# RL-VIG/LibContinual

Hardware: AMD Instinct MI355X
Metric: images/sec/node (task-0 epoch), CIFAR-100 B50-5x10 (higher is better)
Workload: dtype bf16; 1 GPU; lwf_resnet18_b50_task0; method=LWF, backbone=resnet18, per_gpu_batch=256, global_batch=256, image=3x32x32, parallelism=dp1, optimizer=fused SGD

## Files before the change

### libcontinual_amd/csrc/api.hip

```cpp
#include <map>
#include <utility>
#include <vector>
#include <mutex>
#include <string>
#include <string.h>
#include <stdio.h>
#include <stdlib.h>

#include "kernels.h"

static thread_local char g_err[512] = "";

void clhip_set_error(const char* fmt, ...) {
    va_list ap;
    va_start(ap, fmt);
    vsnprintf(g_err, sizeof(g_err), fmt, ap);
    va_end(ap);
}

extern "C" const char* clhip_last_error(void) { return g_err; }
extern "C" int clhip_version(void) { return 103; }

namespace {
const char* const kKeys[] = {
    "ATTN_GENERIC", "ATTN_BWD", "BN_FUSE", "BN_FUSE_MAX_M", "BN_MASK_BITS", "BN_MASK_FROM_Y", "BN_PARTIALS", "CE_ROWS", "CE_ONE_WG", "LINEAR_BWD_SPLIT", "CONV3G", "CONV4", "CONV_V1",
    "GEMM_NO_SPLIT", "GEMM_TAIL", "NO_CONV16", "NO_CONV3", "NO_PARITY_DGRAD", "NO_SHORTCUT", "NO_STEM", "PREP_NARROW", "WGRAD4",
    "WGRAD_NO_TR", "WGRAD2_ATOMIC", "WGRAD_DEFER", "WGRAD_DEFER_SIDE", "BWD_FUSED", "WGRAD_STREAM", "BRANCH_STREAM", "WGRAD_ALWAYS_QUEUE", "SIDE_PRIO", "EVENT_FLAGS", "EVENT_RECORD", "CONV5", "CONV6", "WGRAD16_PARTS", "WGRAD32_IPG", "WGRAD64_IPG", "WGRAD64_IPI2", "CONV64", "CONV64_BM", "CONV64_FWD", "CONV6_PAIR", "CONV7", "CONV7_TPW", "WGRAD7", "FWD7", "PAIR_BN_FUSE", "POOL_BN_FUSE", "BN_INPUT", "BN_INPUT_WT", "BN_RES_INPUT", "BN_GRAD", "BN_GRAD_MINC", "BN_GRAD_RES", "CONV6_DEBUG", "BN_ONEPASS", "WGRAD5", "WGRAD32",
    "BN_ACC_CPT", "BN_BWD_ITERS", "CONV3_CFG", "CONV4_CFG", "CONV4_GRID", "GEMM_GROUP_M", "GEMM_MT", "IGEMM_TILE",
    "SHORTCUT_MIN_PIXELS", "STEM_GRID", "STEM_WGRAD_GRID", "WGRAD4_MIN_STEPS", "WGRAD4_MIN_TOTAL", "WGRAD_NET_GFLOP", "WGRAD_TARGET",
    "CONV5_MIN_TILES", "CONV5_GRID", "CONV64_MAX_W", "CONV64_MAX_M", "CONV8", "CONV8_MIN_TILES", "DZ_BUFFERS", "CONV8_GRID", "CONV8_OPT", "CONV8_BNR", "CONV9", "PLAN_SKIP", "WT_DEBUG", "EVAL_LAZY", "GEMM_SPLITK", "STREAM_PROBE", "STAGE_EVAL", "STAGE_TRAIN", "STAGE_TRAIN_BWD", "STAGE_TRACE", "STAGE_ENTRY", "STAGE_ENTRY_BWD", "STAGE_POOL", "STAGE_XCH3", "ADAPTER_TM",
    "CONV3_DEBUG", "WGRAD_DEBUG", "CONV4_FORCE_CFG", "CONV4_ENABLE", "CONV4_DEBUG", "CONV4_TRACE", "WGRAD4_TRACE", "CONV6_TRACE", "CONV8_TRACE", "CONV9_TRACE",
};
std::mutex g_stream_mu;
std::mutex g_cfg_mu;
std::map<std::string, const char*>& cfg_map() { static std::map<std::string, const char*> m; return m; }
bool known_key(const char* k) {
    for (const char* q : kKeys) if (strcmp(q, k) == 0) return true;
    return false;
}
}

namespace {
__global__ void stream_probe_spin_kernel(unsigned long long* out, long long ticks) {
    const unsigned long long t0 = wall_clock64();
    while ((long long)(wall_clock64() - t0) < ticks) __builtin_amdgcn_s_sleep(64);
    out[0] = wall_clock64();
}
__global__ void stream_probe_stamp_kernel(unsigned long long* out) { out[1] = wall_clock64(); }

struct SharedStreams {
    std::vector<hipStream_t> pool;
    std::map<std::pair<hipStream_t, int>, hipStream_t> chosen;
    hipStream_t low_prio = nullptr;
    unsigned long long* probe_buf = nullptr;
};
SharedStreams g_shared[16];

bool runs_beside(SharedStreams& S, hipStream_t a, hipStream_t b) {
    if (S.probe_buf == nullptr && hipMalloc(reinterpret_cast<void**>(&S.probe_buf), 2 * sizeof(unsigned long long)) != hipSuccess) return false;
    hipLaunchKernelGGL(stream_probe_spin_kernel, dim3(1), dim3(1), 0, a, S.probe_buf, 30000ll);
    hipLaunchKernelGGL(stream_probe_stamp_kernel, dim3(1), dim3(1), 0, b, S.probe_buf);
    if (hipStreamSynchronize(b) != hipSuccess || hipStreamSynchronize(a) != hipSuccess) return false;
    unsigned long long h[2] = {0, 0};
// ... 106 lines not shown
```

### libcontinual_amd/csrc/conv.hip

```cpp
#include <stdlib.h>

#include <algorithm>

#include "kernels.h"

namespace {

constexpr int BK = 32;

struct ConvParams {
    const void* src;
    const void* wt;
    void* dst;
    float* stats;
    int N, Hs, Ws, Cs, log2Cs, Hd, Wd, Cd, ksize, stride, pad, accumulate;
    int M;
    int K;
};

template <typename T> struct Chunk;
template <> struct Chunk<bf16_t> { uint4 a; };
template <> struct Chunk<float> { uint4 a, b; };

template <typename T> __device__ __forceinline__ Chunk<T> zero_chunk() {
// ... 361 lines not shown
    int BN = Cd >= 128 ? 128 : (Cd >= 64 ? 64 : (Cd >= 32 ? 32 : 16));
    int gy = (Cd + BN - 1) / BN;
    bool small = ((int64_t)((M + 127) / 128) * gy) < 512;
    return small ? 64 : 128;
}

int check_conv(int N, int H, int W, int C, int K, int ksize, int stride, int pad) {
    CLHIP_CHECK_ARG(N > 0 && H > 0 && W > 0);
    CLHIP_CHECK_ARG(ksize == 1 || ksize == 3);
    CLHIP_CHECK_ARG(stride >= 1 && pad >= 0);
    CLHIP_CHECK_ARG(C >= 8 && ilog2_exact(C) >= 0);
    CLHIP_CHECK_ARG(K >= 16 && K % 16 == 0);
    CLHIP_CHECK_ARG((int64_t)N * H * W * (C > K ? C : K) < (int64_t)1 << 31);
    return CLHIP_OK;
}

}

static bool use_v3() {
    static const bool v = clhip_cfg("NO_CONV3") == nullptr;
    return v;
}
static bool use_v1() {
    static const bool v = clhip_cfg("CONV_V1") != nullptr;
    return v;
}

extern "C" int clhip_conv_fwd_tiles(int N, int H, int W, int C, int K, int ksize, int stride, int pad) {
    int Ho = (H + 2 * pad - ksize) / stride + 1, Wo = (W + 2 * pad - ksize) / stride + 1;
    int M = N * Ho * Wo;
    if (ksize == 7) return clhip_stem7_supported(N, H, W, C, K, stride, pad) ? clhip_stem7_fwd_tiles(N, H, W) : 0;
    if (!use_v1()) {
        int t2 = clhip_conv2_tiles_m(M, K);
        if (use_v3() && clhip_conv16_supported(H, W, C, K, ksize, stride, pad, CLHIP_BF16)) {
            int t16 = clhip_conv16_tiles_m(M);
            return t16 > t2 ? t16 : t2;
        }
        if (use_v3() && clhip_conv3_supported(H, W, C, K, ksize, stride, pad, CLHIP_BF16)) {
            int t3 = clhip_conv3_tiles_m(M, K);
            if (clhip_conv4_supported(N, H, W, C, K, ksize, stride, pad, CLHIP_BF16)) { int t4 = clhip_conv4_tiles_m(M, C, K, W); if (t4 > t3) t3 = t4; }
            return t3 > t2 ? t3 : t2;
        }
        return t2;
    }
    int bm = fwd_tile_m(M, K);
    return (M + bm - 1) / bm;
}

static bool conv64_fwd_on() { const char* c = clhip_cfg("CONV64_FWD"); return !(c != nullptr && atoi(c) == 0); }

static bool wgrad_v1_no_tr() { static const bool v = clhip_cfg("WGRAD_NO_TR") != nullptr; return v; }

enum { OP_FWD = 0, OP_DGRAD = 1, OP_WGRAD = 2, OP_DGRAD_BNR = 3, OP_FWD_WT = 4 };
static int route_conv(int op, int form, int N, int H, int W, int C, int Creal, int K, int ksize, int stride, int pad, int dtype) {
    CLHIP_CHECK_ARG(op >= OP_FWD && op <= OP_FWD_WT);
    CLHIP_CHECK_ARG(form >= 0 && form <= (op == OP_FWD ? 2 : (op == OP_WGRAD ? 1 : 0)));
    if (ksize == 7 && (op == OP_FWD || op == OP_WGRAD)) {
        CLHIP_CHECK_ARG(clhip_stem7_supported(N, H, W, C, K, stride, pad));
        if (op == OP_FWD) CLHIP_CHECK_ARG(form != 1);
        else CLHIP_CHECK_ARG(form == 1 && Creal >= 1 && Creal <= C && (K * 49 * Creal) % 4 == 0);
        CLHIP_CHECK_ARG(dtype == CLHIP_BF16 || dtype == CLHIP_F32);
        return op == OP_FWD ? CLHIP_CONV_STEM7 : CLHIP_CONV_WGRAD_STEM7;
    }
    if (int e = check_conv(N, H, W, C, K, ksize, stride, pad)) return e;
    const bool v2 = !use_v1();
    const bool v3 = v2 && use_v3();
    if (op == OP_FWD) {
        CLHIP_CHECK_ARG(!(form == 2 && !v2));
        CLHIP_CHECK_ARG(dtype == CLHIP_BF16 || dtype == CLHIP_F32);
        const bool rows = form == 1;
        if (v3 && !rows && clhip_stem_supported(N, H, W, C, K, ksize, stride, pad, dtype)) return CLHIP_CONV_STEM;
        if (v3 && !rows && conv64_fwd_on() && clhip_conv64_supported(N, H, W, C, K, ksize, stride, pad, dtype)) return CLHIP_CONV_CONV64;
        if (v3 && clhip_conv16_supported(H, W, C, K, ksize, stride, pad, dtype)) return CLHIP_CONV_CONV16;
        if (v3 && !rows && clhip_conv8_supported(N, H, W, C, K, ksize, stride, pad, dtype)) return CLHIP_CONV_CONV8;
        if (v3 && !rows && clhip_conv5_supported(N, H, W, C, K, ksize, stride, pad, dtype)) return CLHIP_CONV_CONV5;
        if (v3 && !rows && clhip_conv9_supported(N, H, W, C, K, ksize, stride, pad, dtype)) return CLHIP_CONV_CONV9;
        if (v3 && clhip_conv4_supported(N, H, W, C, K, ksize, stride, pad, dtype)) return CLHIP_CONV_CONV4;
        if (v3 && clhip_conv3_supported(H, W, C, K, ksize, stride, pad, dtype)) return CLHIP_CONV_CONV3;
        return v2 ? CLHIP_CONV_CONV2 : CLHIP_CONV_V1;
    }
    if (op == OP_DGRAD) {
        CLHIP_CHECK_ARG(C % 16 == 0);
        CLHIP_CHECK_ARG(ilog2_exact(K) >= 0);
        CLHIP_CHECK_ARG(dtype == CLHIP_BF16 || dtype == CLHIP_F32);
        if (v3 && clhip_shortcut_supported(N, H, W, C, K, ksize, stride, pad, dtype)) return CLHIP_CONV_SHORTCUT;
        if (v3 && clhip_conv16_supported(H, W, K, C, ksize, stride, pad, dtype)) return CLHIP_CONV_CONV16;
        if (v3 && clhip_conv64_supported(N, H, W, K, C, ksize, stride, pad, dtype)) return CLHIP_CONV_CONV64;
        if (v3 && clhip_conv8_supported(N, H, W, K, C, ksize, stride, pad, dtype)) return CLHIP_CONV_CONV8;
        if (v3 && clhip_conv5_supported(N, H, W, K, C, ksize, stride, pad, dtype)) return CLHIP_CONV_CONV5;
        if (v3 && clhip_conv9_supported(N, H, W, K, C, ksize, stride, pad, dtype)) return CLHIP_CONV_CONV9;
        if (v3 && clhip_conv4_supported(N, H, W, K, C, ksize, stride, pad, dtype)) return CLHIP_CONV_CONV4;
        if (v3 && clhip_conv3_supported(H, W, K, C, ksize, stride, pad, dtype)) return CLHIP_CONV_CONV3;
        return v2 ? CLHIP_CONV_CONV2 : CLHIP_CONV_V1;
    }
    if (op == OP_WGRAD) {
        CLHIP_CHECK_ARG(Creal >= 1 && Creal <= C);
        CLHIP_CHECK_ARG(dtype == CLHIP_BF16 || dtype == CLHIP_F32);
        const bool ws = form == 1;
        if (v3 && ws && clhip_stem_wgrad_supported(N, H, W, C, Creal, K, ksize, stride, pad, dtype)) return CLHIP_CONV_WGRAD_STEM;
        if (v3 && ws && clhip_wgrad64_supported(N, H, W, C, Creal, K, ksize, stride, pad, dtype)) return CLHIP_CONV_WGRAD64;
        if (v3 && ws && clhip_wgrad4_supported(N, H, W, C, Creal, K, ksize, stride, pad, dtype)) return CLHIP_CONV_WGRAD4;
        if (v3 && clhip_wgrad3_supported(N, H, W, C, Creal, K, ksize, stride, pad, dtype)) return CLHIP_CONV_WGRAD3;
        if (v3 && ws && clhip_wgrad16_supported(N, H, W, C, Creal, K, ksize, stride, pad, dtype)) return CLHIP_CONV_WGRAD16;
        if (v3 && ws && clhip_wgrad32_supported(N, H, W, C, Creal, K, ksize, stride, pad, dtype)) return CLHIP_CONV_WGRAD32;
        if (v2) return (ws && clhip_wgrad2_ws_bytes(N, H, W, C, Creal, K, ksize, stride, pad) > 0) ? CLHIP_CONV_WGRAD2_DET : CLHIP_CONV_WGRAD2_ATOMIC;
        return (dtype == CLHIP_BF16 && !wgrad_v1_no_tr()) ? CLHIP_CONV_WGRAD_V1 : CLHIP_CONV_WGRAD_V1_NO_TR;
    }
    if (op == OP_DGRAD_BNR) {
        CLHIP_CHECK_ARG(v3 && (clhip_conv16_supported(H, W, K, C, ksize, stride, pad, dtype) || clhip_conv64_supported(N, H, W, K, C, ksize, stride, pad, dtype) ||
                               clhip_conv8_supported(N, H, W, K, C, ksize, stride, pad, dtype) || clhip_conv4_supported(N, H, W, K, C, ksize, stride, pad, dtype)));
// ... 33 lines not shown
}

static int conv_fwd_impl(const void* x, const void* w_fwd, void* z, float* stat_partials, double* stat_acc, int stat_rep, int N, int H, int W, int C,
                         int K, int ksize, int stride, int pad, int dtype, void* stream) {
    const int family = route_conv(OP_FWD, stat_partials ? 1 : (stat_acc ? 2 : 0), N, H, W, C, C, K, ksize, stride, pad, dtype);
    if (family < 0) return family;
    CLHIP_CHECK_ARG(x && w_fwd && z);
    hipStream_t st = static_cast<hipStream_t>(stream);
    if (family == CLHIP_CONV_STEM7) return clhip_stem7_fwd_launch(x, w_fwd, z, stat_acc, stat_rep, N, H, W, K, dtype, st);
    ConvParams p;
    p.src = x; p.wt = w_fwd; p.dst = z; p.stats = stat_partials;
    p.N = N; p.Hs = H; p.Ws = W; p.Cs = C; p.log2Cs = ilog2_exact(C);
    p.Hd = (H + 2 * pad - ksize) / stride + 1; p.Wd = (W + 2 * pad - ksize) / stride + 1; p.Cd = K;
    p.ksize = ksize; p.stride = stride; p.pad = pad; p.accumulate = 0;
    p.M = N * p.Hd * p.Wd; p.K = ksize * ksize * C;
    ConvCall c;
    c.src = x; c.wt = w_fwd; c.dst = z; c.stats = stat_partials; c.stat_acc = stat_acc; c.stat_rep = stat_rep;
    c.N = N; c.H = H; c.W = W; c.Cs = C; c.Cd = K;
    auto zero_tail = [&](int tiles_used) {
        const int tiles_alloc = clhip_conv_fwd_tiles(N, H, W, C, K, ksize, stride, pad);
        if (stat_partials && tiles_alloc > tiles_used)
            hipMemsetAsync(stat_partials + (size_t)tiles_used * 2 * K, 0, (size_t)(tiles_alloc - tiles_used) * 2 * K * sizeof(float), st);
    };
    switch (family) {
        case CLHIP_CONV_STEM: return clhip_stem_launch(x, w_fwd, z, stat_acc, stat_rep, N, H, W, K, st);
        case CLHIP_CONV_CONV64: return clhip_conv64_launch(c, st);
        case CLHIP_CONV_CONV16:
            zero_tail(clhip_conv16_tiles_m(p.M));
            return clhip_conv16_launch(c, st);
        case CLHIP_CONV_CONV8: return clhip_conv8_launch(c, st);
        case CLHIP_CONV_CONV5: return clhip_conv5_launch(c, st);
        case CLHIP_CONV_CONV9: return clhip_conv9_launch(c, st);
        case CLHIP_CONV_CONV4:
            zero_tail(clhip_conv4_tiles_m(p.M, C, K, W));
            return clhip_conv4_launch(c, st);
        case CLHIP_CONV_CONV3:
            zero_tail(clhip_conv3_tiles_m(p.M, K));
            return clhip_conv3_launch(c, st);
        case CLHIP_CONV_CONV2:
            zero_tail(clhip_conv2_tiles_m(p.M, K));
            return clhip_conv2_launch(x, w_fwd, z, stat_partials, stat_acc, stat_rep, N, H, W, C, p.Hd, p.Wd, K, ksize, stride, pad, 0, 0, dtype, st);
        case CLHIP_CONV_V1: return dtype == CLHIP_BF16 ? launch_igemm<bf16_t, 0>(p, st) : launch_igemm<float, 0>(p, st);
        default: break;
    }
    clhip_set_error("clhip_conv_fwd: no launch for kernel family %d", family);
    return CLHIP_EINVAL;
}

extern "C" int clhip_conv_dgrad(const void* dz, const void* w_dg, void* dx, int accumulate, int N, int H, int W, int C,
                                int K, int ksize, int stride, int pad, int dtype, void* stream) {
    const int family = route_conv(OP_DGRAD, 0, N, H, W, C, C, K, ksize, stride, pad, dtype);
    if (family < 0) return family;
    CLHIP_CHECK_ARG(dz && w_dg && dx);
    ConvParams p;
    p.src = dz; p.wt = w_dg; p.dst = dx; p.stats = nullptr;
    p.N = N; p.Hs = (H + 2 * pad - ksize) / stride + 1; p.Ws = (W + 2 * pad - ksize) / stride + 1; p.Cs = K;
    p.log2Cs = ilog2_exact(K);
    p.Hd = H; p.Wd = W; p.Cd = C;
    p.ksize = ksize; p.stride = stride; p.pad = pad; p.accumulate = accumulate;
    p.M = N * H * W; p.K = ksize * ksize * K;
    ConvCall c;
    c.src = dz; c.wt = w_dg; c.dst = dx; c.N = N; c.H = H; c.W = W; c.Cs = K; c.Cd = C; c.accumulate = accumulate; c.mode = 1;
    hipStream_t st = static_cast<hipStream_t>(stream);
    switch (family) {
        case CLHIP_CONV_SHORTCUT: return clhip_shortcut_dgrad(dz, w_dg, dx, accumulate, N, H, W, C, K, st);
        case CLHIP_CONV_CONV16: return clhip_conv16_launch(c, st);
        case CLHIP_CONV_CONV64: return clhip_conv64_launch(c, st);
// ... 310 lines not shown
```

### libcontinual_amd/csrc/conv4.hip

```cpp
#include <stdlib.h>

#include "kernels.h"

namespace {

int g_force4[4] = {0, 0, 0, 0};
int g_enable4 = -1, g_debug4 = 0;
unsigned long long* g_trace4 = nullptr;

typedef __attribute__((ext_vector_type(16))) float f32x16;
typedef __attribute__((ext_vector_type(4))) unsigned u32x4;
typedef __attribute__((address_space(1))) const void gvoid_t;
typedef __attribute__((address_space(3))) void lvoid_t;

struct Conv4Params {
    const bf16_t* src;
    const bf16_t* wt;
    bf16_t* dst;
    float* stats;
    double* stat_acc;
    int stat_rep;
    const bf16_t* bn_z;
    const bf16_t* bn_y;
    const float* bn_mean;
    const float* bn_invstd;
    double* bn_acc;
    int bn_rep;
    int H, W, Cs, Cd, M, accumulate;
    int wshift, hshift;
    int np;
    int patch_bytes;
    int n_ntiles, nt_shift, n_items;
    int cpg;
    unsigned long long* trace;
    int debug;
};

template <int MODE>
__device__ __forceinline__ unsigned tap_mask4(int g, const Conv4Params& p) {
    int w, h;
    if (p.wshift >= 0 && p.hshift >= 0) { w = g & (p.W - 1); h = (g >> p.wshift) & (p.H - 1); }
    else { w = g % p.W; h = (g / p.W) % p.H; }
    constexpr unsigned UP = MODE == 0 ? 0x007u : 0x1c0u, DOWN = MODE == 0 ? 0x1c0u : 0x007u;
    constexpr unsigned LEFT = MODE == 0 ? 0x049u : 0x124u, RIGHT = MODE == 0 ? 0x124u : 0x049u;
    unsigned m = 0x1ffu;
    if (h == 0) m &= ~UP;
    if (h == p.H - 1) m &= ~DOWN;
    if (w == 0) m &= ~LEFT;
    if (w == p.W - 1) m &= ~RIGHT;
    return m;
}

#ifdef CLHIP_ABLATION
#define DBG(p) ((p).debug)
#define STAMP() do { if (p.trace && blockIdx.x == 0 && lane == 0 && (wave & 3) == 0 && nstamp < 256) p.trace[(wave >> 2) * 256 + nstamp++] = __builtin_amdgcn_s_memtime(); } while (0)
#else
#define STAMP() do { } while (0)
#define DBG(p) 0
#endif

template <int N> __device__ __forceinline__ void wait_vm() { __builtin_amdgcn_s_waitcnt((N & 15) | 0x70 | 0xF00 | ((N >> 4) << 14)); }
__device__ __forceinline__ void wait_lds() { __builtin_amdgcn_s_waitcnt(0xC07F); }
__device__ __forceinline__ void wg_barrier(bool skip = false) {
    wait_lds();
    if (!skip) __builtin_amdgcn_s_barrier();
    asm volatile("" ::: "memory");
}

template <int WM, int WN, int KG, int CK, int WMAX, int MODE>
__global__ __launch_bounds__(WM * WN * KG * 64, 2) void conv4_kernel(const Conv4Params p) {
    constexpr int BM = WM * 64, BN = WN * 64, NWG = WM * WN, NTG = NWG * 64;
    constexpr int NST = 3;
    constexpr int PP = CK * 2 + 16;
    constexpr int KS = CK / 16;
    constexpr int WROW = CK * 2;
    constexpr int SPR = WROW / 16;
    constexpr int RPI = 64 / SPR;
    constexpr int SLAB = BN * WROW;
    constexpr int WINST = (BN / RPI) / NWG;
    static_assert((BN / RPI) % NWG == 0 && WINST >= 1, "ring rows must divide among the waves of a group");
    constexpr int SPP = PP / 16;
    constexpr int ZBYTES = 512;
    constexpr int PINST = ((((BM + 2 * WMAX + 2) * PP + 255) / 256 * 256 + ZBYTES) / 1024 + 1 + NWG - 1) / NWG;
    constexpr int PL_TAP = 2;
    constexpr bool SETPRIO = false;
    constexpr bool STAG = NWG * KG == 8;

    extern __shared__ __attribute__((aligned(16))) char smem[];
    const int tid = threadIdx.x, lane = tid & 63;
    const int wave = __builtin_amdgcn_readfirstlane(tid >> 6);
    const int grp = wave / NWG, wv = wave % NWG;
    int nstamp = 0; (void)nstamp;
    const int wm = wv / WN, wn = wv % WN;
    const int l31 = lane & 31, kh = lane >> 5;
    const int W = p.W, Cs = p.Cs, halo = W + 1;
    const int K9 = 9 * Cs;

    char* patch_g = smem + grp * 2 * p.patch_bytes;
    char* ring0 = smem + KG * 2 * p.patch_bytes;
    char* ring_g = ring0 + grp * SLAB;
    constexpr int XR_BYTES = KG > 1 ? (KG - 1) * NWG * 64 * 64 * 4 : 0;
    const int ring_end = KG * 2 * p.patch_bytes + NST * KG * SLAB;
    float* red = reinterpret_cast<float*>(smem + (ring_end > XR_BYTES ? ring_end : XR_BYTES));

    int xaddr[2];
#pragma unroll
    for (int i = 0; i < 2; ++i) xaddr[i] = (wm * 64 + i * 32 + l31 + halo) * PP + kh * 16;
    const int zoff = (p.np * PP + 255) / 256 * 256;
    int waddr[2][KS];
#pragma unroll
    for (int j = 0; j < 2; ++j) {
        const int o = wn * 64 + j * 32 + l31;
        const int swz = CK == 64 ? ((o >> 1) & 7) : ((o >> 2) & 3);
#pragma unroll
        for (int ks = 0; ks < KS; ++ks) waddr[j][ks] = o * WROW + (((2 * ks + kh) ^ swz) << 4);
    }
    unsigned dma_lane[WINST];
#pragma unroll
    for (int i = 0; i < WINST; ++i) {
        const int row = (wv * WINST + i) * RPI + lane / SPR;
        const int slot = lane % SPR;
        const int swz = CK == 64 ? ((row >> 1) & 7) : ((row >> 2) & 3);
        dma_lane[i] = (unsigned)((row * K9 + (slot ^ swz) * 8) * 2);
    }
    const char* wbase = reinterpret_cast<const char*>(p.wt);
    auto dma = [&](int item, int cc, int tap, int stage) {
        const int n0 = (item & (p.n_ntiles - 1)) * BN;
        const size_t uni = ((size_t)n0 * K9 + (size_t)tap * Cs + (size_t)(grp * p.cpg + cc) * CK) * 2;
        const char* g = wbase + uni;
        char* l = ring_g + stage * (KG * SLAB) + wv * (WINST * 1024);
        if (DBG(p) & 2) return;
#if defined(__HIP_DEVICE_COMPILE__)
#pragma unroll
        for (int i = 0; i < WINST; ++i)
            __builtin_amdgcn_global_load_lds((gvoid_t*)(g + dma_lane[i]), (lvoid_t*)(l + i * 1024), 16, 0, 0);
#else
        (void)g; (void)l;
#endif
    };

    const __amdgpu_buffer_rsrc_t srs = __builtin_amdgcn_make_buffer_rsrc(const_cast<bf16_t*>(p.src), 0, p.M * Cs * 2, 0x00020000);
    constexpr int OOB = 0x40000000;
    int prel[PINST];
#pragma unroll
    for (int i = 0; i < PINST; ++i) {
        const int slot = (wv * PINST + i) * 64 + lane;
        const int q = slot / SPP, sub = slot - q * SPP;
        prel[i] = (q < p.np && sub < SPP - 1) ? q * (Cs * 2) + sub * 16 : OOB;
    }
    auto pdma = [&](int item, int cc, int buf) {
        const int m0 = (item >> p.nt_shift) * BM;
        const int base = (m0 - halo) * (Cs * 2) + (grp * p.cpg + cc) * CK * 2;
        char* l = patch_g + buf * p.patch_bytes + wv * (PINST * 1024);
#if defined(__HIP_DEVICE_COMPILE__)
#pragma unroll
        for (int i = 0; i < PINST; ++i)
            __builtin_amdgcn_raw_ptr_buffer_load_lds(srs, (lvoid_t*)(l + i * 1024), 16, prel[i] + base, 0, 0, 0);
#else
        (void)base; (void)l;
#endif
    };

    const int G = gridDim.x;
    const int nmy = (p.n_items - (int)blockIdx.x + G - 1) / G;
    const int cpg = p.cpg;

    const bool pl_on = !(DBG(p) & 4);
    if (pl_on) pdma(blockIdx.x, 0, 0);
    dma(blockIdx.x, 0, 0, 0);
    dma(blockIdx.x, 0, 1, 1);
    if constexpr (STAG) {
        wait_vm<WINST>();
    } else {
        dma(blockIdx.x, 0, 2, 2);
        wait_vm<2 * WINST>();
    }
    wg_barrier();

    constexpr int UK = STAG ? KS : KS / 2;
    bf16x8_t ax[UK][2], aw[UK][2], bx[UK][2], bw[UK][2];
    int cur = 0;
    for (int k = 0; k < nmy; ++k) {
        const int item = blockIdx.x + k * G;
        const int m0 = (item >> p.nt_shift) * BM, n0 = (item & (p.n_ntiles - 1)) * BN;
        unsigned tmask[2];
#pragma unroll
        for (int i = 0; i < 2; ++i) {
            const int g = m0 + wm * 64 + i * 32 + l31;
            tmask[i] = g < p.M ? tap_mask4<MODE>(g, p) : 0u;
        }
        auto frags = [&](bf16x8_t (&xf)[UK][2], bf16x8_t (&wf)[UK][2], const char* pb, int r, int s, int u) {
            if (DBG(p) & 64) return;
            const char* ws = ring_g + s * (KG * SLAB);
            const int shift = (MODE == 0 ? (r - 1) * W + (s - 1) : (1 - r) * W + (1 - s)) * PP;
            const unsigned bit = 1u << (3 * r + s);
            int xa[2];
#pragma unroll
            for (int i = 0; i < 2; ++i) { const int a = xaddr[i] + shift; xa[i] = (tmask[i] & bit) ? a : zoff + (a & 255); }
#pragma unroll
            for (int q = 0; q < UK; ++q) {
#pragma unroll
                for (int i = 0; i < 2; ++i) xf[q][i] = *reinterpret_cast<const bf16x8_t*>(pb + xa[i] + (u * UK + q) * 32);
#pragma unroll
                for (int j = 0; j < 2; ++j) wf[q][j] = *reinterpret_cast<const bf16x8_t*>(ws + waddr[j][u * UK + q]);
            }
        };
        f32x16 acc[2][2];
#pragma unroll
        for (int j = 0; j < 2; ++j)
#pragma unroll
            for (int i = 0; i < 2; ++i)
#pragma unroll
                for (int r = 0; r < 16; ++r) acc[j][i][r] = 0.f;
        auto mma = [&](const bf16x8_t (&xf)[UK][2], const bf16x8_t (&wf)[UK][2]) {
            if (DBG(p) & 1) {
#pragma unroll
                for (int q = 0; q < UK; ++q)
#pragma unroll
                    for (int j = 0; j < 2; ++j) asm volatile("" ::"v"(xf[q][j]), "v"(wf[q][j]));
                return;
            }
#pragma unroll
            for (int q = 0; q < UK; ++q)
#pragma unroll
                for (int j = 0; j < 2; ++j)
#pragma unroll
                    for (int i = 0; i < 2; ++i) acc[j][i] = __builtin_amdgcn_mfma_f32_32x32x16_bf16(wf[q][j], xf[q][i], acc[j][i], 0, 0, 0);
// ... 198 lines not shown
                        for (int g4 = 0; g4 < 4; ++g4) {
                            const int cc2 = wn * 64 + j * 32 + g4 * 8 + kh * 4;
                            const float* v = sv + which * 16 + g4 * 4;
                            *reinterpret_cast<f32x4*>(red + ((wm * 2 + rh) * 2 + which) * BN + cc2) = f32x4{v[0], v[1], v[2], v[3]};
                        }
                }
            }
            wg_barrier();
            for (int idx = tid; idx < 2 * BN; idx += NTG) {
                const int which = idx / BN, c2 = idx - which * BN;
                float t = 0.f;
#pragma unroll
                for (int w2 = 0; w2 < WM * 2; ++w2) t += red[(w2 * 2 + which) * BN + c2];
                const int mt = item >> p.nt_shift;
                if (MODE == 0) {
                    if (p.stat_acc != nullptr) atomicAdd(p.stat_acc + ((size_t)(mt & (p.stat_rep - 1)) * 2 + which) * p.Cd + n0 + c2, (double)t);
                    else p.stats[((size_t)mt * 2 + which) * p.Cd + n0 + c2] = t;
                } else {
                    if (which == 1) {
                        float sg = 0.f;
#pragma unroll
                        for (int w2 = 0; w2 < WM * 2; ++w2) sg += red[(w2 * 2 + 0) * BN + c2];
                        t = p.bn_invstd[n0 + c2] * (t - p.bn_mean[n0 + c2] * sg);
                    }
                    atomicAdd(p.bn_acc + ((size_t)(mt & (p.bn_rep - 1)) * 2 + which) * p.Cd + n0 + c2, (double)t);
                }
            }
        }
    }
}

struct Cfg4 { int wm, wn, kg, ck; };

template <int WM, int WN, int KG, int CK, int WMAX, int MODE>
int launch4(Conv4Params& p, hipStream_t st) {
    constexpr int BM = WM * 64, BN = WN * 64, PP = CK * 2 + 16, NWG = WM * WN;
    p.np = BM + 2 * p.W + 2;
    p.patch_bytes = (((((BM + 2 * WMAX + 2) * PP + 255) / 256 * 256 + 512) / 1024 + 1 + NWG - 1) / NWG) * NWG * 1024;
    p.n_ntiles = p.Cd / BN;
    p.nt_shift = ilog2_exact(p.n_ntiles);
    const int n_mtiles = (p.M + BM - 1) / BM;
    p.n_items = n_mtiles * p.n_ntiles;
    p.cpg = (p.Cs / CK) / KG;
    size_t lds = (size_t)KG * 2 * p.patch_bytes + (size_t)3 * KG * BN * CK * 2;
    if (KG > 1) { size_t x = (size_t)(KG - 1) * NWG * 64 * 64 * sizeof(float); if (x > lds) lds = x; }
    lds += (size_t)WM * 2 * 2 * BN * sizeof(float);
    if (lds > 160 * 1024) { clhip_set_error("conv4: %zu bytes of LDS", lds); return CLHIP_EINVAL; }
    auto kern = conv4_kernel<WM, WN, KG, CK, WMAX, MODE>;
    static size_t attr = 0;
    if (lds > attr) {
        if (hipFuncSetAttribute(reinterpret_cast<const void*>(kern), hipFuncAttributeMaxDynamicSharedMemorySize, (int)lds) != hipSuccess) {
            clhip_set_error("conv4: cannot reserve %zu bytes of LDS", lds);
            return CLHIP_EHIP;
        }
        attr = lds;
    }
    int per_cu = (int)((160 * 1024) / lds);
    const int wave_cap = 8 / (NWG * KG) > 0 ? 8 / (NWG * KG) : 1;
    if (per_cu > wave_cap) per_cu = wave_cap;
    if (per_cu < 1) per_cu = 1;
    static const int force_grid = clhip_cfg("CONV4_GRID") ? atoi(clhip_cfg("CONV4_GRID")) : 0;
    int grid = 256 * per_cu;
    if (force_grid > 0) grid = force_grid;
    if (KG > 1 || grid > p.n_items) grid = p.n_items;
    hipLaunchKernelGGL(kern, dim3(grid), dim3(NWG * KG * 64), lds, st, p);
    CLHIP_LAUNCH_CHECK();
    return CLHIP_OK;
}

Cfg4 pick4(int M, int Cs, int Cd, int W) {
    static const char* ov = clhip_cfg("CONV4_CFG");
    if (g_force4[0] > 0) return Cfg4{g_force4[0], g_force4[1], g_force4[2], g_force4[3]};
    if (ov) { Cfg4 c{0, 0, 0, 0}; if (sscanf(ov, "%d,%d,%d,%d", &c.wm, &c.wn, &c.kg, &c.ck) == 4) return c; }
    auto tiles = [&](int bm, int bn) { return (int64_t)((M + bm - 1) / bm) * (Cd / bn); };
    if (Cd % 128 == 0 && tiles(256, 128) >= 200) return Cfg4{4, 2, 1, 64};
    if (Cd % 128 == 0 && tiles(128, 128) >= 200 && (Cs / 32) % 2 == 0) return Cfg4{2, 2, 2, 32};
    if (tiles(256, 64) >= 256) return Cfg4{4, 1, 1, 32};
    if (tiles(64, 64) <= 256 && (Cs / 32) % 4 == 0 && W <= 16) return Cfg4{1, 1, 4, 32};
    if (W <= 8 && tiles(128, 64) >= 128 && (Cs / 64) % 2 == 0) return Cfg4{2, 1, 2, 64};
    if ((Cs / 32) % 2 == 0) return Cfg4{2, 1, 2, 32};
    return Cfg4{2, 1, 1, 32};
}

bool cfg_ok(const Cfg4& c, int Cs, int Cd) {
    if (!(c.ck == 32 || c.ck == 64)) return false;
    if (Cs % c.ck || Cd % (c.wn * 64)) return false;
    if ((Cs / c.ck) % c.kg) return false;
    const int nt = Cd / (c.wn * 64);
    return (nt & (nt - 1)) == 0;
}

}

bool clhip_conv4_supported(int N, int H, int W, int Cs, int Cd, int ksize, int stride, int pad, int dtype) {
    static const bool on = clhip_cfg("CONV4") ? atoi(clhip_cfg("CONV4")) != 0 : true;
    if (g_enable4 >= 0 ? g_enable4 == 0 : !on) return false;
    if (!(dtype == CLHIP_BF16 && ksize == 3 && stride == 1 && pad == 1 && (Cs % 64) == 0 && (Cd % 64) == 0 && W <= 32 && W >= 2 && H >= 1)) return false;
    if ((int64_t)N * H * W * (Cs > Cd ? Cs : Cd) * 2 >= ((int64_t)1 << 29)) return false;
    const int nt = Cd / 64;
    return (nt & (nt - 1)) == 0;
}

int clhip_conv4_tiles_m(int M, int Cs, int Cd, int W) { return (M + pick4(M, Cs, Cd, W).wm * 64 - 1) / (pick4(M, Cs, Cd, W).wm * 64); }

int clhip_conv4_launch(const ConvCall& c, hipStream_t st) {
    const BnSums none, &b = c.bnr ? *c.bnr : none;
    CLHIP_CHECK_ARG(c.in == nullptr && c.bn_in == nullptr && c.rs == nullptr && !(b.mask || b.gamma || b.beta || b.coef));
    const int W = c.W, Cs = c.Cs, Cd = c.Cd, mode = c.mode;
    Conv4Params p;
    p.bn_z = static_cast<const bf16_t*>(b.z); p.bn_y = static_cast<const bf16_t*>(b.y); p.bn_mean = b.mean; p.bn_invstd = b.invstd;
    p.bn_acc = b.acc; p.bn_rep = b.rep > 0 ? b.rep : 1;
    p.src = static_cast<const bf16_t*>(c.src); p.wt = static_cast<const bf16_t*>(c.wt); p.dst = static_cast<bf16_t*>(c.dst);
    p.stats = c.stats; p.stat_acc = c.stat_acc; p.stat_rep = c.stat_rep > 0 ? c.stat_rep : 1;
    p.H = c.H; p.W = W; p.wshift = ilog2_exact(W); p.hshift = ilog2_exact(c.H); p.Cs = Cs; p.Cd = Cd; p.accumulate = c.accumulate; p.M = c.N * c.H * W;
    p.debug = g_debug4; p.trace = g_trace4;
    Cfg4 g = pick4(p.M, Cs, Cd, W);
    if (!cfg_ok(g, Cs, Cd)) { clhip_set_error("conv4: configuration %d,%d,%d,%d does not fit Cs=%d Cd=%d", g.wm, g.wn, g.kg, g.ck, Cs, Cd); return CLHIP_EINVAL; }
#define L4(a, b, g, k) (W <= 8 ? (mode == 0 ? launch4<a, b, g, k, 8, 0>(p, st) : launch4<a, b, g, k, 8, 1>(p, st)) \
                               : (mode == 0 ? launch4<a, b, g, k, 32, 0>(p, st) : launch4<a, b, g, k, 32, 1>(p, st)))
    const int key = g.wm * 1000 + g.wn * 100 + g.kg * 10 + (g.ck == 64 ? 1 : 0);
    switch (key) {
        case 4110: return L4(4, 1, 1, 32);
        case 4111: return L4(4, 1, 1, 64);
        case 2110: return L4(2, 1, 1, 32);
        case 2111: return L4(2, 1, 1, 64);
        case 2210: return L4(2, 2, 1, 32);
        case 2211: return L4(2, 2, 1, 64);
        case 4210: return L4(4, 2, 1, 32);
        case 4211: return L4(4, 2, 1, 64);
        case 2120: return L4(2, 1, 2, 32);
        case 2121: return L4(2, 1, 2, 64);
        case 1220: return L4(1, 2, 2, 32);
        case 2220: return L4(2, 2, 2, 32);
        case 1140: return L4(1, 1, 4, 32);
        case 1141: return L4(1, 1, 4, 64);
        case 2140: return L4(2, 1, 4, 32);
        case 2141: return L4(2, 1, 4, 64);
        case 1240: return L4(1, 2, 4, 32);
        default: break;
    }
#undef L4
    clhip_set_error("conv4: no kernel for configuration %d,%d,%d,%d", g.wm, g.wn, g.kg, g.ck);
    return CLHIP_EINVAL;
}

void clhip_conv4_set_cfg(int wm, int wn, int kg, int ck) { g_force4[0] = wm; g_force4[1] = wn; g_force4[2] = kg; g_force4[3] = ck; }
void clhip_conv4_enable(int on) { g_enable4 = on; }
void clhip_conv4_set_debug(int bits) { g_debug4 = bits; }
// ... 2 lines not shown
```

### libcontinual_amd/csrc/kernels.h

```cpp
#pragma once
#include "common.h"

struct BnSums {
    const void* z = nullptr;
    const void* y = nullptr;
    const void* mask = nullptr;
    const float* gamma = nullptr; const float* beta = nullptr;
    const float* mean = nullptr; const float* invstd = nullptr;
    const float* coef = nullptr;
    double* acc = nullptr;
    int rep = 1;
};

struct ConvCall {
    const void* src = nullptr;
    const void* wt = nullptr;
    void* dst = nullptr;
    float* stats = nullptr;
    double* stat_acc = nullptr;
    int stat_rep = 1;
    int N = 0, H = 0, W = 0, Cs = 0, Cd = 0;
    int accumulate = 0;
    int mode = 0;
    const LazyIn* in = nullptr;
    const clhip_bn_input* bn_in = nullptr;
    const clhip_bn_res_input* rs = nullptr;
    const BnSums* bnr = nullptr;
};

void clhip_bn_set_fwd_stop_event(hipEvent_t ev);
void clhip_bn_set_stop_event(hipEvent_t ev);
hipEvent_t clhip_bn_pending_stop_event();

int clhip_conv2_tiles_m(int M, int Cd);
int clhip_conv2_launch(const void* src, const void* wt, void* dst, float* stats, double* stat_acc, int stat_rep, int N, int Hs, int Ws, int Cs, int Hd, int Wd,
                       int Cd, int ksize, int stride, int pad, int accumulate, int mode, int dtype, hipStream_t st);
size_t clhip_wgrad2_ws_bytes(int N, int H, int W, int C, int Creal, int K, int ksize, int stride, int pad);
int clhip_wgrad2_launch(const void* x, const void* dz, float* dw, float* ws, int N, int H, int W, int C, int Creal, int K, int ksize, int stride,
                        int pad, int dtype, hipStream_t st);

bool clhip_conv16_supported(int H, int W, int Cs, int Cd, int ksize, int stride, int pad, int dtype);
int clhip_conv16_tiles_m(int M);
int clhip_conv16_launch(const ConvCall& c, hipStream_t st);
bool clhip_conv64_supported(int N, int H, int W, int Cs, int Cd, int ksize, int stride, int pad, int dtype);
int clhip_conv64_launch(const ConvCall& c, hipStream_t st);
bool clhip_conv3_supported(int H, int W, int Cs, int Cd, int ksize, int stride, int pad, int dtype);
int clhip_conv3_tiles_m(int M, int Cd);
int clhip_conv3_launch(const ConvCall& c, hipStream_t st);
bool clhip_wgrad32_supported(int N, int H, int W, int C, int Creal, int K, int ksize, int stride, int pad, int dtype);
size_t clhip_wgrad32_ws_bytes(int N);
int clhip_wgrad32_launch(const void* x, const void* dz, float* dw, float* ws, int N, int H, const float* x_coef, hipStream_t st);
bool clhip_wgrad64_supported(int N, int H, int W, int C, int Creal, int K, int ksize, int stride, int pad, int dtype);
size_t clhip_wgrad64_ws_bytes(int N);
int clhip_wgrad64_launch(const void* x, const void* dz, float* dw, float* ws, int N, int H, const float* x_coef, hipStream_t st);
bool clhip_wgrad16_supported(int N, int H, int W, int C, int Creal, int K, int ksize, int stride, int pad, int dtype);
size_t clhip_wgrad16_ws_bytes(int N);
int clhip_wgrad16_launch(const void* x, const void* dz, float* dw, float* ws, int N, int H, const float* x_coef, hipStream_t st);
bool clhip_wgrad3_supported(int N, int H, int W, int C, int Creal, int K, int ksize, int stride, int pad, int dtype);
size_t clhip_wgrad3_ws_bytes(int N, int H, int W, int C, int K);
int clhip_wgrad3_launch(const void* x, const void* dz, float* dw, float* ws, int N, int H, int W, int C, int Creal, int K, hipStream_t st);
bool clhip_bwd_fused_supported(int N, int H, int W, int C, int Creal, int K, int ksize, int stride, int pad, int dtype);
int clhip_bwd_fused_launch(const void* x, const void* dz, const void* w_dg, void* dx, int accumulate, float* dw, float* ws, int N, int H, int W, int C,
                           const BnSums& bnr, const float* x_coef, const clhip_bn_grad* lz, hipStream_t st);
void clhip_wgrad_defer_begin();
void clhip_wgrad_defer_abort();
void clhip_wgrad_defer_pause(bool paused);
int clhip_wgrad_defer_flush(hipStream_t st, bool end);
int clhip_wgrad_reduce_launch(const float* slab, float* dw, int64_t n4, int splits, hipStream_t st);

bool clhip_conv4_supported(int N, int H, int W, int Cs, int Cd, int ksize, int stride, int pad, int dtype);
int clhip_conv4_tiles_m(int M, int Cs, int Cd, int W);
int clhip_conv4_launch(const ConvCall& c, hipStream_t st);
void clhip_conv4_set_cfg(int wm, int wn, int kg, int ck);
void clhip_conv4_enable(int on);
void clhip_conv4_set_debug(int bits);
void clhip_conv4_set_trace(unsigned long long* dev_buf);

bool clhip_conv5_supported(int N, int H, int W, int Cs, int Cd, int ksize, int stride, int pad, int dtype);
void clhip_conv5_enable(int on);
void clhip_conv5_min_tiles(int n);
int clhip_conv5_tiles_m(int M);
int clhip_conv5_launch(const ConvCall& c, hipStream_t st);

bool clhip_dgrad6_supported(int N, int H, int W, int C, int K, int dtype);
void clhip_conv6_enable(int on);
void clhip_conv6_set_trace(unsigned long long* buf, int wg);
size_t clhip_dgrad6_packed_bytes(int C, int K);
int clhip_dgrad6_pack(const void* w_dg, const void* w_sc_dg, void* packed, int C, int K, hipStream_t st);
int clhip_dgrad6_launch(const void* dz, const void* w_packed, const void* dz_sc, void* dx, int accumulate, int N, int H, int W, int C, int K, hipStream_t st);

bool clhip_dgrad7_supported(int N, int H, int W, int C, int K, int dtype);
size_t clhip_dgrad7_packed_bytes(int C, int K);
int clhip_dgrad7_pack(const void* w_dg, const void* w_sc_dg, void* packed, int C, int K, hipStream_t st);
int clhip_dgrad7_launch(const void* dz, const void* w_packed, const void* dz_sc, void* dx, int accumulate, int N, int H, int W, int C, int K, hipStream_t st,
                        const void* bn_z = nullptr, const void* bn_y = nullptr, const float* bn_mean = nullptr, const float* bn_invstd = nullptr, double* bn_acc = nullptr,
                        int bn_rep = 1);
bool clhip_wgrad7_supported(int N, int H, int W, int C, int K, int dtype);
size_t clhip_wgrad7_ws_bytes(int N, int C, int K, int which);
int clhip_wgrad7_launch(const void* x, const void* dz, const void* dz_sc, float* dw, float* dw_sc, float* ws3, float* ws_sc, int N, int C, hipStream_t st);
bool clhip_fwd7_supported(int N, int H, int W, int C, int K, int dtype);
int clhip_fwd7_launch(const void* x, const void* w3, const void* wsc, void* z3, void* zsc, double* acc3, int rep3, double* accsc, int repsc, int N, int H, int W, int C,
                      hipStream_t st);

bool clhip_conv8_supported(int N, int H, int W, int Cs, int Cd, int ksize, int stride, int pad, int dtype);
void clhip_conv8_enable(int on);
// ... 53 lines not shown
```

Measured before the change: 125,900 images/sec.

## Add stride-2 forward path to conv4 implicit-GEMM kernel

Extends the conv4 implicit-GEMM kernel with a stride-2 template variant. It gathers the four parity planes of the input into the LDS patch and remaps tap shifts and boundary masks to match. Dispatch routes eligible stride-2 3x3 forward convs (Cs>=128, enough tiles) to this kernel instead of the older conv3/conv2 paths, aiming for better MFMA utilisation on downsampling layers. This adds a larger LDS patch and new indexing that could be mis-tuned.

Result: no change. 126,400 images/sec (median of 4 runs) (+0.4%).

```diff
diff --git a/libcontinual_amd/csrc/api.hip b/libcontinual_amd/csrc/api.hip
--- a/libcontinual_amd/csrc/api.hip
+++ b/libcontinual_amd/csrc/api.hip
@@ -28,7 +28,7 @@
     "WGRAD_NO_TR", "WGRAD2_ATOMIC", "WGRAD_DEFER", "WGRAD_DEFER_SIDE", "BWD_FUSED", "WGRAD_STREAM", "BRANCH_STREAM", "WGRAD_ALWAYS_QUEUE", "SIDE_PRIO", "EVENT_FLAGS", "EVENT_RECORD", "CONV5", "CONV6", "WGRAD16_PARTS", "WGRAD32_IPG", "WGRAD64_IPG", "WGRAD64_IPI2", "CONV64", "CONV64_BM", "CONV64_FWD", "CONV6_PAIR", "CONV7", "CONV7_TPW", "WGRAD7", "FWD7", "PAIR_BN_FUSE", "POOL_BN_FUSE", "BN_INPUT", "BN_INPUT_WT", "BN_RES_INPUT", "BN_GRAD", "BN_GRAD_MINC", "BN_GRAD_RES", "CONV6_DEBUG", "BN_ONEPASS", "WGRAD5", "WGRAD32",
     "BN_ACC_CPT", "BN_BWD_ITERS", "CONV3_CFG", "CONV4_CFG", "CONV4_GRID", "GEMM_GROUP_M", "GEMM_MT", "IGEMM_TILE",
     "SHORTCUT_MIN_PIXELS", "STEM_GRID", "STEM_WGRAD_GRID", "WGRAD4_MIN_STEPS", "WGRAD4_MIN_TOTAL", "WGRAD_NET_GFLOP", "WGRAD_TARGET",
-    "CONV5_MIN_TILES", "CONV5_GRID", "CONV64_MAX_W", "CONV64_MAX_M", "CONV8", "CONV8_MIN_TILES", "DZ_BUFFERS", "CONV8_GRID", "CONV8_OPT", "CONV8_BNR", "CONV9", "PLAN_SKIP", "WT_DEBUG", "EVAL_LAZY", "GEMM_SPLITK", "STREAM_PROBE", "STAGE_EVAL", "STAGE_TRAIN", "STAGE_TRAIN_BWD", "STAGE_TRACE", "STAGE_ENTRY", "STAGE_ENTRY_BWD", "STAGE_POOL", "STAGE_XCH3", "ADAPTER_TM",
+    "CONV5_MIN_TILES", "CONV4_S2_MIN_TILES", "CONV5_GRID", "CONV64_MAX_W", "CONV64_MAX_M", "CONV8", "CONV8_MIN_TILES", "DZ_BUFFERS", "CONV8_GRID", "CONV8_OPT", "CONV8_BNR", "CONV9", "PLAN_SKIP", "WT_DEBUG", "EVAL_LAZY", "GEMM_SPLITK", "STREAM_PROBE", "STAGE_EVAL", "STAGE_TRAIN", "STAGE_TRAIN_BWD", "STAGE_TRACE", "STAGE_ENTRY", "STAGE_ENTRY_BWD", "STAGE_POOL", "STAGE_XCH3", "ADAPTER_TM",
     "CONV3_DEBUG", "WGRAD_DEBUG", "CONV4_FORCE_CFG", "CONV4_ENABLE", "CONV4_DEBUG", "CONV4_TRACE", "WGRAD4_TRACE", "CONV6_TRACE", "CONV8_TRACE", "CONV9_TRACE",
 };
 std::mutex g_stream_mu;
diff --git a/libcontinual_amd/csrc/conv.hip b/libcontinual_amd/csrc/conv.hip
--- a/libcontinual_amd/csrc/conv.hip
+++ b/libcontinual_amd/csrc/conv.hip
@@ -417,6 +417,7 @@
     if (ksize == 7) return clhip_stem7_supported(N, H, W, C, K, stride, pad) ? clhip_stem7_fwd_tiles(N, H, W) : 0;
     if (!use_v1()) {
         int t2 = clhip_conv2_tiles_m(M, K);
+        if (use_v3() && clhip_conv4_s2_shape_ok(N, H, W, C, K, ksize, stride, pad, CLHIP_BF16)) { int t4 = clhip_conv4_s2_tiles_m(N, H, W, C, K); if (t4 > t2) t2 = t4; }
         if (use_v3() && clhip_conv16_supported(H, W, C, K, ksize, stride, pad, CLHIP_BF16)) {
             int t16 = clhip_conv16_tiles_m(M);
             return t16 > t2 ? t16 : t2;
@@ -461,6 +462,7 @@
         if (v3 && !rows && clhip_conv5_supported(N, H, W, C, K, ksize, stride, pad, dtype)) return CLHIP_CONV_CONV5;
         if (v3 && !rows && clhip_conv9_supported(N, H, W, C, K, ksize, stride, pad, dtype)) return CLHIP_CONV_CONV9;
         if (v3 && clhip_conv4_supported(N, H, W, C, K, ksize, stride, pad, dtype)) return CLHIP_CONV_CONV4;
+        if (v3 && clhip_conv4_s2_supported(N, H, W, C, K, ksize, stride, pad, dtype)) return CLHIP_CONV_CONV4;
         if (v3 && clhip_conv3_supported(H, W, C, K, ksize, stride, pad, dtype)) return CLHIP_CONV_CONV3;
         return v2 ? CLHIP_CONV_CONV2 : CLHIP_CONV_V1;
     }
@@ -560,7 +562,8 @@
         case CLHIP_CONV_CONV5: return clhip_conv5_launch(c, st);
         case CLHIP_CONV_CONV9: return clhip_conv9_launch(c, st);
         case CLHIP_CONV_CONV4:
-            zero_tail(clhip_conv4_tiles_m(p.M, C, K, W));
+            c.stride = stride;
+            zero_tail(stride == 2 ? clhip_conv4_s2_tiles_m(N, H, W, C, K) : clhip_conv4_tiles_m(p.M, C, K, W));
             return clhip_conv4_launch(c, st);
         case CLHIP_CONV_CONV3:
             zero_tail(clhip_conv3_tiles_m(p.M, K));
diff --git a/libcontinual_amd/csrc/conv4.hip b/libcontinual_amd/csrc/conv4.hip
--- a/libcontinual_amd/csrc/conv4.hip
+++ b/libcontinual_amd/csrc/conv4.hip
@@ -29,6 +29,8 @@
     int H, W, Cs, Cd, M, accumulate;
     int wshift, hshift;
     int np;
+    int src_pixels;
+    int Wi;
     int patch_bytes;
     int n_ntiles, nt_shift, n_items;
     int cpg;
@@ -36,7 +38,7 @@
     int debug;
 };
 
-template <int MODE>
+template <int MODE, int S2 = 0>
 __device__ __forceinline__ unsigned tap_mask4(int g, const Conv4Params& p) {
     int w, h;
     if (p.wshift >= 0 && p.hshift >= 0) { w = g & (p.W - 1); h = (g >> p.wshift) & (p.H - 1); }
@@ -45,9 +47,9 @@
     constexpr unsigned LEFT = MODE == 0 ? 0x049u : 0x124u, RIGHT = MODE == 0 ? 0x124u : 0x049u;
     unsigned m = 0x1ffu;
     if (h == 0) m &= ~UP;
-    if (h == p.H - 1) m &= ~DOWN;
+    if (!S2 && h == p.H - 1) m &= ~DOWN;
     if (w == 0) m &= ~LEFT;
-    if (w == p.W - 1) m &= ~RIGHT;
+    if (!S2 && w == p.W - 1) m &= ~RIGHT;
     return m;
 }
 
@@ -67,8 +69,9 @@
     asm volatile("" ::: "memory");
 }
 
-template <int WM, int WN, int KG, int CK, int WMAX, int MODE>
+template <int WM, int WN, int KG, int CK, int WMAX, int MODE, int S2 = 0>
 __global__ __launch_bounds__(WM * WN * KG * 64, 2) void conv4_kernel(const Conv4Params p) {
+    static_assert(!S2 || MODE == 0, "the stride-2 patch exists for the forward only");
     constexpr int BM = WM * 64, BN = WN * 64, NWG = WM * WN, NTG = NWG * 64;
     constexpr int NST = 3;
     constexpr int PP = CK * 2 + 16;
@@ -81,7 +84,9 @@
     static_assert((BN / RPI) % NWG == 0 && WINST >= 1, "ring rows must divide among the waves of a group");
     constexpr int SPP = PP / 16;
     constexpr int ZBYTES = 512;
-    constexpr int PINST = ((((BM + 2 * WMAX + 2) * PP + 255) / 256 * 256 + ZBYTES) / 1024 + 1 + NWG - 1) / NWG;
+    constexpr int S2W = 16, NP0 = BM + 1, NP1 = BM + S2W + 1;
+    constexpr int NPMAX = S2 ? 2 * NP0 + 2 * NP1 : BM + 2 * WMAX + 2;
+    constexpr int PINST = (((NPMAX * PP + 255) / 256 * 256 + ZBYTES) / 1024 + 1 + NWG - 1) / NWG;
     constexpr int PL_TAP = 2;
     constexpr bool SETPRIO = false;
     constexpr bool STAG = NWG * KG == 8;
@@ -105,7 +110,7 @@
 
     int xaddr[2];
 #pragma unroll
-    for (int i = 0; i < 2; ++i) xaddr[i] = (wm * 64 + i * 32 + l31 + halo) * PP + kh * 16;
+    for (int i = 0; i < 2; ++i) xaddr[i] = (wm * 64 + i * 32 + l31 + (S2 ? 0 : halo)) * PP + kh * 16;
     const int zoff = (p.np * PP + 255) / 256 * 256;
     int waddr[2][KS];
 #pragma unroll
@@ -139,18 +144,27 @@
 #endif
     };
 
-    const __amdgpu_buffer_rsrc_t srs = __builtin_amdgcn_make_buffer_rsrc(const_cast<bf16_t*>(p.src), 0, p.M * Cs * 2, 0x00020000);
+    const __amdgpu_buffer_rsrc_t srs = __builtin_amdgcn_make_buffer_rsrc(const_cast<bf16_t*>(p.src), 0, p.src_pixels * Cs * 2, 0x00020000);
     constexpr int OOB = 0x40000000;
     int prel[PINST];
 #pragma unroll
     for (int i = 0; i < PINST; ++i) {
         const int slot = (wv * PINST + i) * 64 + lane;
         const int q = slot / SPP, sub = slot - q * SPP;
-        prel[i] = (q < p.np && sub < SPP - 1) ? q * (Cs * 2) + sub * 16 : OOB;
+        if constexpr (S2) {
+            const int pl = (q >= NP0) + (q >= 2 * NP0) + (q >= 2 * NP0 + NP1);
+            const int pr = pl >> 1, pc = pl & 1;
+            const int u = q - (pr ? 2 * NP0 + pc * NP1 + S2W + 1 : pc * NP0 + 1);
+            const int jr = u >> p.wshift, c = u & (W - 1);
+            const bool ok = q < NPMAX && sub < SPP - 1 && u >= (pr ? -W : 0);
+            prel[i] = ok ? ((2 * jr + pr) * p.Wi + 2 * c + pc) * (Cs * 2) + sub * 16 : OOB;
+        } else {
+            prel[i] = (q < p.np && sub < SPP - 1) ? q * (Cs * 2) + sub * 16 : OOB;
+        }
     }
     auto pdma = [&](int item, int cc, int buf) {
         const int m0 = (item >> p.nt_shift) * BM;
-        const int base = (m0 - halo) * (Cs * 2) + (grp * p.cpg + cc) * CK * 2;
+        const int base = (S2 ? 4 * m0 : m0 - halo) * (Cs * 2) + (grp * p.cpg + cc) * CK * 2;
         char* l = patch_g + buf * p.patch_bytes + wv * (PINST * 1024);
 #if defined(__HIP_DEVICE_COMPILE__)
 #pragma unroll
@@ -187,12 +201,13 @@
 #pragma unroll
         for (int i = 0; i < 2; ++i) {
             const int g = m0 + wm * 64 + i * 32 + l31;
-            tmask[i] = g < p.M ? tap_mask4<MODE>(g, p) : 0u;
+            tmask[i] = g < p.M ? tap_mask4<MODE, S2>(g, p) : 0u;
         }
         auto frags = [&](bf16x8_t (&xf)[UK][2], bf16x8_t (&wf)[UK][2], const char* pb, int r, int s, int u) {
             if (DBG(p) & 64) return;
             const char* ws = ring_g + s * (KG * SLAB);
-            const int shift = (MODE == 0 ? (r - 1) * W + (s - 1) : (1 - r) * W + (1 - s)) * PP;
+            const int shift = (S2 ? (r == 1 ? (s != 1) * NP0 + 1 : 2 * NP0 + (s != 1) * NP1 + S2W + 1 - (r == 0 ? W : 0)) - (s == 0)
+                                  : (MODE == 0 ? (r - 1) * W + (s - 1) : (1 - r) * W + (1 - s))) * PP;
             const unsigned bit = 1u << (3 * r + s);
             int xa[2];
 #pragma unroll
@@ -457,11 +472,12 @@
 
 struct Cfg4 { int wm, wn, kg, ck; };
 
-template <int WM, int WN, int KG, int CK, int WMAX, int MODE>
+template <int WM, int WN, int KG, int CK, int WMAX, int MODE, int S2 = 0>
 int launch4(Conv4Params& p, hipStream_t st) {
     constexpr int BM = WM * 64, BN = WN * 64, PP = CK * 2 + 16, NWG = WM * WN;
-    p.np = BM + 2 * p.W + 2;
-    p.patch_bytes = (((((BM + 2 * WMAX + 2) * PP + 255) / 256 * 256 + 512) / 1024 + 1 + NWG - 1) / NWG) * NWG * 1024;
+    constexpr int NPMAX = S2 ? 4 * BM + 36 : BM + 2 * WMAX + 2;
+    p.np = S2 ? NPMAX : BM + 2 * p.W + 2;
+    p.patch_bytes = ((((NPMAX * PP + 255) / 256 * 256 + 512) / 1024 + 1 + NWG - 1) / NWG) * NWG * 1024;
     p.n_ntiles = p.Cd / BN;
     p.nt_shift = ilog2_exact(p.n_ntiles);
     const int n_mtiles = (p.M + BM - 1) / BM;
@@ -471,7 +487,7 @@
     if (KG > 1) { size_t x = (size_t)(KG - 1) * NWG * 64 * 64 * sizeof(float); if (x > lds) lds = x; }
     lds += (size_t)WM * 2 * 2 * BN * sizeof(float);
     if (lds > 160 * 1024) { clhip_set_error("conv4: %zu bytes of LDS", lds); return CLHIP_EINVAL; }
-    auto kern = conv4_kernel<WM, WN, KG, CK, WMAX, MODE>;
+    auto kern = conv4_kernel<WM, WN, KG, CK, WMAX, MODE, S2>;
     static size_t attr = 0;
     if (lds > attr) {
         if (hipFuncSetAttribute(reinterpret_cast<const void*>(kern), hipFuncAttributeMaxDynamicSharedMemorySize, (int)lds) != hipSuccess) {
@@ -515,6 +531,36 @@
     return (nt & (nt - 1)) == 0;
 }
 
+Cfg4 pick4_s2(int Cs, int Cd) {
+    if (g_force4[0] > 0) return Cfg4{g_force4[0], g_force4[1], g_force4[2], g_force4[3]};
+    if (Cd % 128 != 0) return Cfg4{2, 1, 1, 32};
+    if (Cs >= 256) return Cfg4{1, 2, 2, 32};
+    return Cfg4{2, 2, 1, 32};
+}
+
+}
+
+bool clhip_conv4_s2_shape_ok(int N, int H, int W, int Cs, int Cd, int ksize, int stride, int pad, int dtype) {
+    static const bool on = clhip_cfg("CONV4") ? atoi(clhip_cfg("CONV4")) != 0 : true;
+    if (g_enable4 >= 0 ? g_enable4 == 0 : !on) return false;
+    if (!(dtype == CLHIP_BF16 && ksize == 3 && stride == 2 && pad == 1 && (Cs % 64) == 0 && (Cd % 64) == 0 && (W == 8 || W == 16 || W == 32) && H >= 2 && H % 2 == 0)) return false;
+    if ((int64_t)N * H * W * Cs * 2 >= ((int64_t)1 << 29) || (int64_t)N * (H / 2) * (W / 2) * Cd * 2 >= ((int64_t)1 << 29)) return false;
+    const int nt = Cd / 64;
+    return (nt & (nt - 1)) == 0;
+}
+
+int clhip_conv4_s2_tiles_m(int N, int H, int W, int Cs, int Cd) {
+    const int bm = pick4_s2(Cs, Cd).wm * 64;
+    return (N * (H / 2) * (W / 2) + bm - 1) / bm;
+}
+
+int clhip_conv4_s2_tiles(int N, int H, int W, int Cs, int Cd) { return clhip_conv4_s2_tiles_m(N, H, W, Cs, Cd) * (Cd / (pick4_s2(Cs, Cd).wn * 64)); }
+
+bool clhip_conv4_s2_supported(int N, int H, int W, int Cs, int Cd, int ksize, int stride, int pad, int dtype) {
+    if (!clhip_conv4_s2_shape_ok(N, H, W, Cs, Cd, ksize, stride, pad, dtype)) return false;
+    const char* v = clhip_cfg("CONV4_S2_MIN_TILES");
+    if (v != nullptr && *v) return clhip_conv4_s2_tiles(N, H, W, Cs, Cd) >= atoi(v);
+    return Cs >= 128 && clhip_conv4_s2_tiles(N, H, W, Cs, Cd) >= 256;
 }
 
 bool clhip_conv4_supported(int N, int H, int W, int Cs, int Cd, int ksize, int stride, int pad, int dtype) {
@@ -531,14 +577,30 @@
 int clhip_conv4_launch(const ConvCall& c, hipStream_t st) {
     const BnSums none, &b = c.bnr ? *c.bnr : none;
     CLHIP_CHECK_ARG(c.in == nullptr && c.bn_in == nullptr && c.rs == nullptr && !(b.mask || b.gamma || b.beta || b.coef));
-    const int W = c.W, Cs = c.Cs, Cd = c.Cd, mode = c.mode;
+    CLHIP_CHECK_ARG(c.stride == 1 || (c.stride == 2 && c.mode == 0 && c.bnr == nullptr && !c.accumulate));
+    const bool s2 = c.stride == 2;
+    const int H = s2 ? c.H / 2 : c.H, W = s2 ? c.W / 2 : c.W, Cs = c.Cs, Cd = c.Cd, mode = c.mode;
     Conv4Params p;
     p.bn_z = static_cast<const bf16_t*>(b.z); p.bn_y = static_cast<const bf16_t*>(b.y); p.bn_mean = b.mean; p.bn_invstd = b.invstd;
     p.bn_acc = b.acc; p.bn_rep = b.rep > 0 ? b.rep : 1;
     p.src = static_cast<const bf16_t*>(c.src); p.wt = static_cast<const bf16_t*>(c.wt); p.dst = static_cast<bf16_t*>(c.dst);
     p.stats = c.stats; p.stat_acc = c.stat_acc; p.stat_rep = c.stat_rep > 0 ? c.stat_rep : 1;
-    p.H = c.H; p.W = W; p.wshift = ilog2_exact(W); p.hshift = ilog2_exact(c.H); p.Cs = Cs; p.Cd = Cd; p.accumulate = c.accumulate; p.M = c.N * c.H * W;
+    p.H = H; p.W = W; p.wshift = ilog2_exact(W); p.hshift = ilog2_exact(H); p.Cs = Cs; p.Cd = Cd; p.accumulate = c.accumulate; p.M = c.N * H * W;
+    p.src_pixels = c.N * c.H * c.W; p.Wi = c.W;
     p.debug = g_debug4; p.trace = g_trace4;
+    if (s2) {
+        CLHIP_CHECK_ARG(clhip_conv4_s2_shape_ok(c.N, c.H, c.W, Cs, Cd, 3, 2, 1, CLHIP_BF16));
+        const Cfg4 g = pick4_s2(Cs, Cd);
+        if (!cfg_ok(g, Cs, Cd)) { clhip_set_error("conv4 (stride 2): configuration %d,%d,%d,%d does not fit Cs=%d Cd=%d", g.wm, g.wn, g.kg, g.ck, Cs, Cd); return CLHIP_EINVAL; }
+        switch (g.wm * 1000 + g.wn * 100 + g.kg * 10 + (g.ck == 64 ? 1 : 0)) {
+            case 2210: return launch4<2, 2, 1, 32, 16, 0, 1>(p, st);
+            case 1220: return launch4<1, 2, 2, 32, 16, 0, 1>(p, st);
+            case 2110: return launch4<2, 1, 1, 32, 16, 0, 1>(p, st);
+            default: break;
+        }
+        clhip_set_error("conv4 (stride 2): no kernel for configuration %d,%d,%d,%d", g.wm, g.wn, g.kg, g.ck);
+        return CLHIP_EINVAL;
+    }
     Cfg4 g = pick4(p.M, Cs, Cd, W);
     if (!cfg_ok(g, Cs, Cd)) { clhip_set_error("conv4: configuration %d,%d,%d,%d does not fit Cs=%d Cd=%d", g.wm, g.wn, g.kg, g.ck, Cs, Cd); return CLHIP_EINVAL; }
 #define L4(a, b, g, k) (W <= 8 ? (mode == 0 ? launch4<a, b, g, k, 8, 0>(p, st) : launch4<a, b, g, k, 8, 1>(p, st)) \
diff --git a/libcontinual_amd/csrc/kernels.h b/libcontinual_amd/csrc/kernels.h
--- a/libcontinual_amd/csrc/kernels.h
+++ b/libcontinual_amd/csrc/kernels.h
@@ -22,6 +22,7 @@
     int N = 0, H = 0, W = 0, Cs = 0, Cd = 0;
     int accumulate = 0;
     int mode = 0;
+    int stride = 1;
     const LazyIn* in = nullptr;
     const clhip_bn_input* bn_in = nullptr;
     const clhip_bn_res_input* rs = nullptr;
@@ -71,6 +72,10 @@
 bool clhip_conv4_supported(int N, int H, int W, int Cs, int Cd, int ksize, int stride, int pad, int dtype);
 int clhip_conv4_tiles_m(int M, int Cs, int Cd, int W);
 int clhip_conv4_launch(const ConvCall& c, hipStream_t st);
+bool clhip_conv4_s2_shape_ok(int N, int H, int W, int Cs, int Cd, int ksize, int stride, int pad, int dtype);
+int clhip_conv4_s2_tiles(int N, int H, int W, int Cs, int Cd);
+int clhip_conv4_s2_tiles_m(int N, int H, int W, int Cs, int Cd);
+bool clhip_conv4_s2_supported(int N, int H, int W, int Cs, int Cd, int ksize, int stride, int pad, int dtype);
 void clhip_conv4_set_cfg(int wm, int wn, int kg, int ck);
 void clhip_conv4_enable(int on);
 void clhip_conv4_set_debug(int bits);
```
